# tum-vision/dvo_slam

Measured on NVIDIA H100. Metric: frame-pair alignments/sec @640x480x5-level, higher is better.
Workload: dtype f32

## Files before the change

### dvo_slam_b200/csrc/stages.cuh

```cuda
#pragma once
#include "common.cuh"
#include "f32x2.cuh"

namespace dvo_b200 {

constexpr unsigned kFullMask = 0xffffffffu;
constexpr int kConsumerWarps = kTileH;
constexpr int kCtaThreads = (kConsumerWarps + 1) * 32;
#ifndef DVO_WIN_COLS
#define DVO_WIN_COLS 152
#endif
#ifndef DVO_WIN_ROWS
#define DVO_WIN_ROWS 24
#endif
#ifndef DVO_STAGES
#define DVO_STAGES 2
#endif
constexpr int kWinCols = DVO_WIN_COLS;
constexpr int kWinRows = DVO_WIN_ROWS;
constexpr int kStages = DVO_STAGES;

__device__ __forceinline__ unsigned smem_u32(const void* p) { return (unsigned)__cvta_generic_to_shared(p); }
__device__ __forceinline__ void mbar_init(unsigned long long* bar, unsigned count) {
  asm volatile("mbarrier.init.shared::cta.b64 [%0], %1;" ::"r"(smem_u32(bar)), "r"(count) : "memory");
}
__device__ __forceinline__ void mbar_fence_init() { asm volatile("fence.mbarrier_init.release.cluster;" ::: "memory"); }
__device__ __forceinline__ void mbar_arrive(unsigned long long* bar) {
  asm volatile("{\n\t.reg .b64 st;\n\tmbarrier.arrive.release.cta.shared::cta.b64 st, [%0];\n\t}" ::"r"(smem_u32(bar)) : "memory");
}
__device__ __forceinline__ void mbar_arrive_expect_tx(unsigned long long* bar, unsigned bytes) {
  asm volatile("{\n\t.reg .b64 st;\n\tmbarrier.arrive.expect_tx.release.cta.shared::cta.b64 st, [%0], %1;\n\t}" ::"r"(smem_u32(bar)),
               "r"(bytes)
               : "memory");
}
#ifndef DVO_TRYWAIT_HINT_NS
#define DVO_TRYWAIT_HINT_NS 0
#endif
__device__ __forceinline__ bool mbar_try_wait(unsigned long long* bar, unsigned parity) {
  unsigned ok;
#if DVO_TRYWAIT_HINT_NS > 0
  asm volatile(
      "{\n\t.reg .pred p;\n\tmbarrier.try_wait.parity.acquire.cta.shared::cta.b64 p, [%1], %2, %3;\n\tselp.u32 %0, 1, 0, p;\n\t}"
      : "=r"(ok)
      : "r"(smem_u32(bar)), "r"(parity), "r"((unsigned)DVO_TRYWAIT_HINT_NS)
      : "memory");
#else
  asm volatile(
      "{\n\t.reg .pred p;\n\tmbarrier.try_wait.parity.acquire.cta.shared::cta.b64 p, [%1], %2;\n\tselp.u32 %0, 1, 0, p;\n\t}"
      : "=r"(ok)
      : "r"(smem_u32(bar)), "r"(parity)
      : "memory");
#endif
  return ok != 0;
}
__device__ __forceinline__ void mbar_wait(unsigned long long* bar, unsigned parity, int* error_flag) {
  unsigned spins = 0;
  while (!mbar_try_wait(bar, parity)) {
    if (((++spins) & 0xfffu) == 0u) {
      if (*reinterpret_cast<volatile int*>(error_flag)) break;
      if (spins > (1u << 24)) { atomicExch(error_flag, 2); break; }
    }
  }
}
__device__ __forceinline__ bool mbar_try_wait_s(unsigned bar, unsigned parity) {
  unsigned ok;
#if DVO_TRYWAIT_HINT_NS > 0
  asm volatile(
      "{\n\t.reg .pred p;\n\tmbarrier.try_wait.parity.acquire.cta.shared::cta.b64 p, [%1], %2, %3;\n\tselp.u32 %0, 1, 0, p;\n\t}"
      : "=r"(ok)
      : "r"(bar), "r"(parity), "r"((unsigned)DVO_TRYWAIT_HINT_NS)
      : "memory");
#else
  asm volatile(
      "{\n\t.reg .pred p;\n\tmbarrier.try_wait.parity.acquire.cta.shared::cta.b64 p, [%1], %2;\n\tselp.u32 %0, 1, 0, p;\n\t}"
      : "=r"(ok)
      : "r"(bar), "r"(parity)
      : "memory");
#endif
  return ok != 0;
}
__device__ __forceinline__ void mbar_wait_s(unsigned bar, unsigned parity, int* error_flag) {
  unsigned spins = 0;
  while (!mbar_try_wait_s(bar, parity)) {
    if (((++spins) & 0xfffu) == 0u) {
      if (*reinterpret_cast<volatile int*>(error_flag)) break;
      if (spins > (1u << 24)) { atomicExch(error_flag, 2); break; }
    }
  }
}
__device__ __forceinline__ void mbar_arrive_s(unsigned bar) {
  asm volatile("{\n\t.reg .b64 st;\n\tmbarrier.arrive.release.cta.shared::cta.b64 st, [%0];\n\t}" ::"r"(bar) : "memory");
}
__device__ __forceinline__ int4 lds_i4(unsigned addr) {
  int4 v;
  asm volatile("ld.shared.v4.b32 {%0, %1, %2, %3}, [%4];" : "=r"(v.x), "=r"(v.y), "=r"(v.z), "=r"(v.w) : "r"(addr));
  return v;
// ... 21 lines not shown
  asm volatile("ld.shared.v2.f32 {%0, %1}, [%2];" : "=f"(v.x), "=f"(v.y) : "r"(addr));
  return v;
}

__device__ __forceinline__ unsigned pin(unsigned v) { asm volatile("" : "+r"(v)); return v; }
__device__ __forceinline__ int pin(int v) { asm volatile("" : "+r"(v)); return v; }
__device__ __forceinline__ float pin(float v) { asm volatile("" : "+f"(v)); return v; }
template <typename T>
__device__ __forceinline__ const T* pin(const T* p) { asm volatile("" : "+l"(p)); return p; }

struct __align__(16) TileDesc {
  int skip;
  int origin;
  int ulo, ucount;
  int vlo, vcount;
  int exact;
  int pad_;
};
struct __align__(128) StageBuf {
  float2 ref0[kTileH][kTileW];
  float tx[kTileW];
  float2 ref1[kTileH][kTileW];
  float2 win[kWinRows][kWinCols];
};
static_assert(offsetof(StageBuf, tx) == kRecTx * sizeof(float2) && offsetof(StageBuf, ref1) == kRecP1 * sizeof(float2) &&
              offsetof(StageBuf, win) == kRecF2 * sizeof(float2), "StageBuf must mirror the reference tile record");
struct TilePipe {
  StageBuf buf[kStages];
  unsigned long long full[kStages], empty[kStages];
  TileDesc desc[kStages];
};
static_assert(sizeof(TileDesc) == 32 && offsetof(TilePipe, desc) % 16 == 0, "TileDesc is read as two 16-byte words");

#ifdef DVO_PIPE_TIMING
struct PipeTiming {
  unsigned long long wait_full_a = 0, wait_full_b = 0, wait_empty = 0, produce = 0, rounds_a = 0, rounds_b = 0;
  unsigned long long tiles = 0, tiles_inexact = 0, tiles_skipped = 0, slow_rounds = 0, rounds = 0;
  bool on = false;
};
#define DVO_CLOCK(tm) ((tm).on ? clock64() : 0)
#define DVO_ADD(tm, field, v) do { if ((tm).on) (tm).field += (v); } while (0)
#else
struct PipeTiming {};
#define DVO_CLOCK(tm) 0ll
#define DVO_ADD(tm, field, v) do { } while (0)
#endif

struct LevelGeom {
  int w, h, n, pitch;
  int nbands, nstrips;
  int strip0, strip_step, nmine;
};

struct StageConsts {
  f2 k0, k1, k2, k3;
  float k8, k9, k10, k11;
  f2 Pa, Pb;
  f2 cgh, cg, fxyh;
  float c_i, ubx, uby;
  int first_iteration;
};

__device__ __forceinline__ void load_stage_consts(const PairState& st, const PairLevel& pl, int w, int h, bool weights_from_prev,
                                                  StageConsts& c) {
  float kt[12], P[4];
#pragma unroll
  for (int i = 0; i < 12; ++i) kt[i] = __ldcg(&st.kt[i]);
#pragma unroll
  for (int i = 0; i < 4; ++i) P[i] = weights_from_prev ? __ldcg(&st.precision_prev[i]) : __ldcg(&st.precision[i]);
  c.k0 = pk(kt[0], kt[4]); c.k1 = pk(kt[1], kt[5]); c.k2 = pk(kt[2], kt[6]); c.k3 = pk(kt[3], kt[7]);
  c.k8 = kt[8]; c.k9 = kt[9]; c.k10 = kt[10]; c.k11 = kt[11];
  c.Pa = pk(P[0], P[1]); c.Pb = pk(P[2], P[3]);
  const float cgx = __fdiv_rn(__fmul_rn(0.5f, pl.cfx), 255.0f), cgy = __fdiv_rn(__fmul_rn(0.5f, pl.cfy), 255.0f);
  c.cg = pk(cgx, cgy);
  c.cgh = pk(0.5f * cgx, 0.5f * cgy);
  c.fxyh = pk(0.5f * pl.cfx, 0.5f * pl.cfy);
  c.c_i = 1.0f / 255.0f;
  c.ubx = pin((float)(w - 2)); c.uby = pin((float)(h - 2));
  c.first_iteration = __ldcg(&st.iteration) == 0;
}

template <bool kStageB>
__device__ __noinline__ void produce_tiles(TilePipe& tp, const PairLevel& pl, const LevelGeom& g, const StageConsts& c, unsigned tbase,
                                           int ntiles, int* error_flag, PipeTiming& tm) {
  const int lane = threadIdx.x & 31, sub = lane >> 3;
  const float2* cur = kStageB ? pl.c3 : pl.c0;
  int s_issue = g.strip0, b_issue = 0;
  for (int i0 = 0; i0 < ntiles; i0 += 4) {
    const long long tp0 = DVO_CLOCK(tm);
    unsigned wordA, wordD;
    {
      const int ii = min(i0 + sub, ntiles - 1);
      const int sd = ii / g.nbands;
      const int s = g.strip0 + sd * g.strip_step, b = ii - sd * g.nbands;
      const int y0 = s * kTileH, rows = min(kTileH, g.h - y0);
      const int x0 = b * kTileW, bw = min(kTileW, g.w - x0);
      const float2 zr = __ldg(pl.rrange + (size_t)s * g.nbands + b);
      const float txc = __ldg(pl.rtmpl + ((lane & 1) ? x0 + bw - 1 : x0));
      const float tyc = __ldg(pl.rtmpl + g.w + ((lane & 2) ? y0 + rows - 1 : y0));
      const bool has_depth = zr.x <= zr.y;
      const float z = (lane & 4) ? zr.y : zr.x;
      const float px = txc * z, py = tyc * z;
      const f2 XY = fma2(c.k0, bc(px), fma2(c.k1, bc(py), fma2(c.k2, bc(z), c.k3)));
      const float Zt = fmaf(c.k8, px, fmaf(c.k9, py, fmaf(c.k10, z, c.k11)));
      const float iz = 1.0f / Zt;
      float umin = lo(XY) * iz, vmin = hi(XY) * iz, umax = umin, vmax = vmin;
      const bool front_lane = Zt > 1e-6f && umin == umin && vmin == vmin;
#pragma unroll
      for (int off = 1; off < 8; off <<= 1) {
        umin = fminf(umin, __shfl_xor_sync(kFullMask, umin, off)); umax = fmaxf(umax, __shfl_xor_sync(kFullMask, umax, off));
        vmin = fminf(vmin, __shfl_xor_sync(kFullMask, vmin, off)); vmax = fmaxf(vmax, __shfl_xor_sync(kFullMask, vmax, off));
      }
      const bool front = ((__ballot_sync(kFullMask, front_lane) >> (sub * 8)) & 0xffu) == 0xffu;
      umin = fmaxf(umin, -8.f); vmin = fmaxf(vmin, -8.f); umax = fminf(umax, (float)g.w + 8.f); vmax = fminf(vmax, (float)g.h + 8.f);
      int skip = 0, exact = 0, ncols = 0, nrows = 0, bx0 = 0, row_lo = 0;
      if (!has_depth) {
        skip = 1;
      } else if (!front) {
      } else if (umax < -1.f || vmax < -1.f || umin > (float)g.w || vmin > (float)g.h) {
        skip = 1;
      } else {
        const int col_lo = max((int)floorf(umin) - 2, 0), col_hi = min((int)floorf(umax) + 3, g.w - 1);
        row_lo = max((int)floorf(vmin) - 2, -1);
        const int row_hi = min((int)floorf(vmax) + 3, g.h);
        bx0 = col_lo & ~1;
        ncols = (col_hi + 2 - bx0) & ~1;
        bool whole = true;
        if (ncols > kWinCols) { bx0 += ((ncols - kWinCols) / 2) & ~1; ncols = kWinCols; whole = false; }
        nrows = row_hi - row_lo + 1;
        if (nrows > kWinRows) { row_lo += (nrows - kWinRows) / 2; nrows = kWinRows; whole = false; }
        if (ncols < 4 || nrows < 4) { ncols = 0; nrows = 0; bx0 = 0; row_lo = 0; }
        else exact = whole ? 1 : 0;
      }
      wordA = (unsigned)skip | ((unsigned)exact << 1) | ((unsigned)ncols << 2) | ((unsigned)nrows << 10);
      wordD = (unsigned)bx0 | ((unsigned)(row_lo + 1) << 16);
    }
    DVO_ADD(tm, produce, DVO_CLOCK(tm) - tp0);
    const int kmax = min(4, ntiles - i0);
    for (int k = 0; k < kmax; ++k) {
      const unsigned t = tbase + (unsigned)(i0 + k);
      const int bufi = t % kStages;
      StageBuf& sb = tp.buf[bufi];
      const unsigned wa = __shfl_sync(kFullMask, wordA, k * 8), wd = __shfl_sync(kFullMask, wordD, k * 8);
      const int s = s_issue, b = b_issue;
      if (++b_issue == g.nbands) { b_issue = 0; s_issue += g.strip_step; }
      const int skip = (int)(wa & 1u), ncols = (int)((wa >> 2) & 0xffu), nrows = (int)(wa >> 10);
      const int win_bx0 = (int)(wd & 0xffffu), win_row_lo = (int)(wd >> 16) - 1;
      TileDesc d;
      d.skip = skip; d.exact = (int)((wa >> 1) & 1u); d.pad_ = 0;
      d.origin = 0; d.ulo = 0; d.ucount = 0; d.vlo = 0; d.vcount = 0;
      if (ncols) {
        d.origin = (win_row_lo * kWinCols + win_bx0) * 8;
        d.ulo = win_bx0 == 0 ? 0 : win_bx0 + 1;
        const int uhi = (win_bx0 + ncols - 1 >= g.w - 1) ? g.w - 2 : win_bx0 + ncols - 3;
        d.ucount = max(uhi - d.ulo + 1, 0);
        d.vlo = win_row_lo + 1;
        d.vcount = max(nrows - 3, 0);
      }
      const unsigned win_row_bytes = (unsigned)ncols * 8u;
      const unsigned rec_bytes = (unsigned)(kStageB ? kRecF2 : kRecP1) * 8u;
      const unsigned total = skip ? 0u : rec_bytes + (unsigned)nrows * win_row_bytes;
      const long long tp1 = DVO_CLOCK(tm);
      mbar_wait(&tp.empty[bufi], ((t / kStages) & 1u) ^ 1u, error_flag);
      DVO_ADD(tm, wait_empty, DVO_CLOCK(tm) - tp1);
      DVO_ADD(tm, tiles, 1); DVO_ADD(tm, tiles_inexact, (!d.skip && !d.exact) ? 1 : 0); DVO_ADD(tm, tiles_skipped, d.skip ? 1 : 0);
      if (lane == 0) {
        tp.desc[bufi] = d;
        if (total) mbar_arrive_expect_tx(&tp.full[bufi], total);
        else mbar_arrive(&tp.full[bufi]);
      }
      __syncwarp();
      if (!skip) {
        if (lane < nrows) {
          const int yy = min(max(win_row_lo + lane, 0), g.h - 1);
          bulk_g2s(&sb.win[lane][0], cur + (size_t)yy * g.pitch + win_bx0, win_row_bytes, &tp.full[bufi]);
        }
        if (lane == 31) bulk_g2s(&sb.ref0[0][0], pl.r0 + (size_t)(s * g.nbands + b) * kRecF2, rec_bytes, &tp.full[bufi]);
      }
    }
  }
}

struct PixelProjection {
  f2 f, gq;
  float Zt;
  int u0, v0;
  bool inb;
};

__device__ __forceinline__ PixelProjection project_pixel(float tx, float ty, float z, const StageConsts& c) {
  PixelProjection p;
  const f2 pxy = mul2(pk(tx, ty), bc(z));
  const float px = lo(pxy), py = hi(pxy);
  const f2 XY = fma2(c.k0, bc(px), fma2(c.k1, bc(py), fma2(c.k2, bc(z), c.k3)));
  p.Zt = __fmaf_rn(c.k8, px, __fmaf_rn(c.k9, py, __fmaf_rn(c.k10, z, c.k11)));
  f2 uv = mul2(XY, bc(rcp_rn(p.Zt)));
  const float u = lo(uv), v = hi(uv);
  p.inb = u >= 0.f && u <= c.ubx && v >= 0.f && v <= c.uby;
  uv = p.inb ? uv : bc(0.f);
  const f2 t = add2_rz(uv, bc(8388608.0f));
  p.f = sub2(uv, sub2(t, bc(8388608.0f)));
  p.gq = sub2(bc(1.0f), p.f);
  p.u0 = __float_as_int(lo(t)) - 0x4b000000;
  p.v0 = __float_as_int(hi(t)) - 0x4b000000;
  return p;
}

#define DVO_BLEND2(fu, fv, gu, gv, c00, c10, c01, c11) \
  fma2(bc(fv), fma2(bc(fu), c11, mul2(bc(gu), c01)), mul2(bc(gv), fma2(bc(fu), c10, mul2(bc(gu), c00))))

__device__ __forceinline__ f2 ld_f2(const float2* p) { const float2 v = *p; return pk(v.x, v.y); }

struct WinView {
  bool exact;
  unsigned base;
  unsigned safe;
  const float2* plane;
  int ulo, ucount, vlo, vcount;
  int w, h, pitch;
};
constexpr int kWinRowBytes = kWinCols * 8;

struct Taps4 { f2 c00, c10, c01, c11; };
struct Taps12 { f2 c00, c10, c01, c11, l0, l1, r0, r1, t0, t1, b0, b1; };

__device__ __forceinline__ void gather_taps4(const WinView& wv, int u0, int v0, bool inb, bool hit, Taps4& t) {
  const bool miss = inb && !hit;
  const unsigned sa = (inb && hit) ? wv.base + (unsigned)(v0 * kWinCols + u0) * 8u : wv.safe;
  const float2* p = miss ? wv.plane + (size_t)v0 * wv.pitch + u0 : reinterpret_cast<const float2*>(__cvta_shared_to_generic(sa));
  const int rp = miss ? wv.pitch : kWinCols;
  t.c00 = ld_f2(p); t.c10 = ld_f2(p + 1); t.c01 = ld_f2(p + rp); t.c11 = ld_f2(p + rp + 1);
}
__device__ __forceinline__ void gather_taps12(const WinView& wv, int u0, int v0, bool inb, bool hit, Taps12& t) {
  const bool miss = inb && !hit;
  const unsigned sa = (inb && hit) ? wv.base + (unsigned)(v0 * kWinCols + u0) * 8u : wv.safe;
  const float2* p = miss ? wv.plane + (size_t)v0 * wv.pitch + u0 : reinterpret_cast<const float2*>(__cvta_shared_to_generic(sa));
  const int rp = miss ? wv.pitch : kWinCols;
  const int up = (miss && v0 == 0) ? 0 : -rp;
  const int dn = (miss && v0 + 2 > wv.h - 1) ? rp : 2 * rp;
  const int dl = u0 > 0 ? 1 : 0, dr = u0 + 2 <= wv.w - 1 ? 2 : 1;
  t.c00 = ld_f2(p); t.c10 = ld_f2(p + 1); t.c01 = ld_f2(p + rp); t.c11 = ld_f2(p + rp + 1);
  t.t0 = ld_f2(p + up); t.t1 = ld_f2(p + up + 1); t.b0 = ld_f2(p + dn); t.b1 = ld_f2(p + dn + 1);
  t.l0 = ld_f2(p - dl); t.l1 = ld_f2(p + rp - dl); t.r0 = ld_f2(p + dr); t.r1 = ld_f2(p + rp + dr);
}

__device__ __forceinline__ float depth_sigma(float z) {
  const float s = __fsub_rn(z, 0.4f);
  return __fmaf_rn(__fmul_rn(0.0019f, s), s, 0.0012f);
}

template <bool kExact>
__device__ __forceinline__ bool residual_pixel(const PixelProjection& p, const WinView& wv, float Ir, float z, const StageConsts& c,
                                               float& ei, float& ez) {
  bool hit = true, any_miss = false;
  if (!kExact && !wv.exact) {
    hit = (unsigned)(p.u0 - wv.ulo) < (unsigned)wv.ucount && (unsigned)(p.v0 - wv.vlo) < (unsigned)wv.vcount;
    any_miss = __any_sync(kFullMask, p.inb && !hit);
  }
  f2 c00, c10, c01, c11;
  if (!any_miss) {
    const unsigned a = p.inb ? wv.base + (unsigned)(p.v0 * kWinCols + p.u0) * 8u : wv.safe;
    c00 = lds_f2<0>(a); c10 = lds_f2<8>(a); c01 = lds_f2<kWinRowBytes>(a); c11 = lds_f2<kWinRowBytes + 8>(a);
  } else {
    Taps4 t;
    gather_taps4(wv, p.u0, p.v0, p.inb, hit, t);
// ... 200 lines not shown
    const f2 ss = pk(s, __int_as_float(__float_as_int(s) ^ st.psign));
    st.acc0 = fma2(ss, bc(st.po0), st.acc0); st.acc1 = fma2(ss, bc(st.po1), st.acc1); st.acc2 = fma2(ss, bc(st.po2), st.acc2);
  }
  const float a0 = xi * xi, a1 = xi * xz, a2 = xz * xz;
  const float s = (v && next) ? w + wn : 0.f;
  const f2 ss = pk(s, __int_as_float(__float_as_int(s) ^ sg));
  st.acc0 = fma2(ss, bc(a0), st.acc0); st.acc1 = fma2(ss, bc(a1), st.acc1); st.acc2 = fma2(ss, bc(a2), st.acc2);
  st.pend = v && !next;
  st.pw = w; st.po0 = a0; st.po1 = a1; st.po2 = a2; st.psign = sg;
  st.cnt += __popc(m);
}

__device__ __forceinline__ void scale_state_export(ScaleState& st, int lane, float* seg_out) {
  float all0 = lo(st.acc0), alt0 = hi(st.acc0), all1 = lo(st.acc1), alt1 = hi(st.acc1), all2 = lo(st.acc2), alt2 = hi(st.acc2);
#pragma unroll
  for (int off = 16; off > 0; off >>= 1) {
    all0 += __shfl_xor_sync(kFullMask, all0, off); alt0 += __shfl_xor_sync(kFullMask, alt0, off);
    all1 += __shfl_xor_sync(kFullMask, all1, off); alt1 += __shfl_xor_sync(kFullMask, alt1, off);
    all2 += __shfl_xor_sync(kFullMask, all2, off); alt2 += __shfl_xor_sync(kFullMask, alt2, off);
  }
  if (lane == 0) {
    seg_out[0] = __int_as_float(st.cnt);
    seg_out[1] = (float)(0.5 * ((double)all0 + (double)alt0)); seg_out[2] = (float)(0.5 * ((double)all1 + (double)alt1));
    seg_out[3] = (float)(0.5 * ((double)all2 + (double)alt2));
    seg_out[4] = (float)(0.5 * ((double)all0 - (double)alt0)); seg_out[5] = (float)(0.5 * ((double)all1 - (double)alt1));
    seg_out[6] = (float)(0.5 * ((double)all2 - (double)alt2));
    seg_out[7] = st.wfirst;
    if (st.cnt == 0) { seg_out[8] = 0.f; seg_out[9] = 0.f; seg_out[10] = 0.f; seg_out[11] = 0.f; }
  }
  if (st.pend) {
    seg_out[8] = st.pw; seg_out[9] = st.po0; seg_out[10] = st.po1; seg_out[11] = st.po2;
  }
}

__device__ __forceinline__ WinView make_view(unsigned bufs, const int4& d0, const int4& d1, const float2* plane, int w, int h, int pitch) {
  WinView wv;
  const unsigned w0 = bufs + (unsigned)offsetof(StageBuf, win);
  wv.base = pin(w0 - (unsigned)d0.y);
  wv.safe = pin(w0 + (unsigned)((kWinCols + 1) * 8));
  wv.plane = plane;
  wv.exact = d1.z != 0;
  wv.ulo = d0.z; wv.ucount = d0.w; wv.vlo = d1.x; wv.vcount = d1.y;
  wv.w = w; wv.h = h; wv.pitch = pitch;
  return wv;
}


template <bool kExact, bool kFirst>
__device__ __forceinline__ void stage_a_rounds(const WinView& wv, int bw, unsigned refa, unsigned txa, float ty, const StageConsts& c,
                                               ScaleState& ss, int lane, unsigned lt_mask) {
  static_assert(kTileW % 64 == 0, "the exact loop takes whole pairs of rounds");
  const int nr = kExact ? kTileW / 32 : (bw + 31) >> 5;
  const int xlim = bw - lane;
  const bool first = kExact ? kFirst : c.first_iteration != 0;
#pragma unroll 1
  for (int r = 0; r < nr; r += 2, refa += 512, txa += 256) {
    const bool second = kExact || r + 1 < nr;
    const f2 rz0 = lds_f2_at(refa);
    const f2 rz1 = second ? lds_f2_at(refa + 256) : pk(0.f, __int_as_float(0x7fc00000));
    const float tx0 = lds_f32(txa), tx1 = second ? lds_f32(txa + 128) : 0.f;
    float z0 = hi(rz0), z1 = hi(rz1);
    if (!kExact && bw < kTileW) {
      z0 = (r * 32 < xlim) ? z0 : __int_as_float(0x7fc00000);
      z1 = (r * 32 + 32 < xlim) ? z1 : __int_as_float(0x7fc00000);
    }
    const PixelProjection p0 = project_pixel(tx0, ty, z0, c);
    const PixelProjection p1 = project_pixel(tx1, ty, z1, c);
    float ei0, ez0, ei1, ez1;
    const bool v0 = residual_pixel<kExact>(p0, wv, lo(rz0), z0, c, ei0, ez0);
    const bool v1 = residual_pixel<kExact>(p1, wv, lo(rz1), z1, c, ei1, ez1);
    const float w0 = student_weight(c, first, ei0, ez0), w1 = student_weight(c, first, ei1, ez1);
    scale_round32(ss, lane, lt_mask, v0, w0, ei0, ez0);
    scale_round32(ss, lane, lt_mask, v1, w1, ei1, ez1);
  }
}
__device__ __forceinline__ void stage_a_run(TilePipe& tp, const PairLevel& pl, const LevelGeom& g, const StageConsts& c,
                                            float* row_exports, unsigned& tile_count, int* error_flag, PipeTiming& tm) {
  const int lane = threadIdx.x & 31, q = threadIdx.x >> 5;
  const unsigned lt_mask = (1u << lane) - 1u;
  const int ntiles = g.nmine * g.nbands;
  const unsigned tbase = tile_count;
  tile_count += ntiles;
  if (q == kConsumerWarps) {
    produce_tiles<false>(tp, pl, g, c, tbase, ntiles, error_flag, tm);
    return;
  }
  int i = 0;
  const unsigned tp_s = pin(smem_u32(&tp));
  const unsigned my_ref = pin((unsigned)(offsetof(StageBuf, ref0) + (q * kTileW + lane) * 8));
  const unsigned my_tx = pin((unsigned)(offsetof(StageBuf, tx) + lane * 4));
  const int gw = pin(g.w), gh = pin(g.h), gnb = pin(g.nbands), gpitch = g.pitch;
  for (int sk = 0, s = g.strip0; sk < g.nmine; ++sk, s += g.strip_step) {
    const int y = s * kTileH + q;
    const bool row_ok = y < gh;
    const float ty = __ldg(pl.rtmpl + gw + min(y, gh - 1));
    ScaleState ss;
    scale_state_init(ss);
    for (int b = 0; b < gnb; ++b, ++i) {
      const unsigned t = tbase + i;
      const unsigned bufi = t % kStages;
      const int x0 = b * kTileW, bw = min(kTileW, gw - x0);
      const long long tw0 = DVO_CLOCK(tm);
      mbar_wait_s(tp_s + (unsigned)offsetof(TilePipe, full) + bufi * 8u, (t / kStages) & 1u, error_flag);
      DVO_ADD(tm, wait_full_a, DVO_CLOCK(tm) - tw0);
      const unsigned bufs = tp_s + bufi * (unsigned)sizeof(StageBuf);
      const int4 d0 = lds_i4(tp_s + (unsigned)offsetof(TilePipe, desc) + bufi * 32u);
      if (row_ok && !d0.x) {
        const int4 d1 = lds_i4(tp_s + (unsigned)offsetof(TilePipe, desc) + bufi * 32u + 16u);
        const WinView wv = make_view(bufs, d0, d1, pl.c0, gw, gh, gpitch);
        const unsigned refa = bufs + my_ref, txa = bufs + my_tx;
        if (wv.exact && bw == kTileW) {
          if (c.first_iteration) stage_a_rounds<true, true>(wv, bw, refa, txa, ty, c, ss, lane, lt_mask);
          else stage_a_rounds<true, false>(wv, bw, refa, txa, ty, c, ss, lane, lt_mask);
        } else {
          stage_a_rounds<false, false>(wv, bw, refa, txa, ty, c, ss, lane, lt_mask);
        }
      }
      __syncwarp();
      if (lane == 0) mbar_arrive_s(tp_s + (unsigned)offsetof(TilePipe, empty) + bufi * 8u);
    }
    if (row_ok) scale_state_export(ss, lane, row_exports + (size_t)y * kSegExportFloats);
  }
}

struct StageBConsts {
  float P00, P01, P10, P11;
  float l, wd0, wd1;
};

constexpr int kNormalValues = 28;

constexpr int kTriValues = 21;
__host__ __device__ constexpr int tri(int r, int c) { return r * 6 - r * (r - 1) / 2 + (c - r); }
struct StageBAcc {
  float A[kTriValues];
  float b[6];
  float llsum;
};

__device__ __forceinline__ void stage_b_init(StageBAcc& a) {
#pragma unroll
  for (int i = 0; i < kTriValues; ++i) a.A[i] = 0.f;
#pragma unroll
  for (int i = 0; i < 6; ++i) a.b[i] = 0.f;
  a.llsum = 0.f;
}

__device__ __forceinline__ void stage_b_rank1(StageBAcc& acc, const f2 V[3], float wd, float s) {
  const float v[6] = {lo(V[0]), hi(V[0]), lo(V[1]), hi(V[1]), lo(V[2]), hi(V[2])};
  float u[6];
#pragma unroll
  for (int r = 0; r < 6; ++r) u[r] = __fmul_rn(v[r], wd);
#pragma unroll
  for (int r = 0; r < 6; ++r) {
#pragma unroll
    for (int c = r; c < 6; ++c) acc.A[tri(r, c)] = __fmaf_rn(u[r], v[c], acc.A[tri(r, c)]);
  }
#pragma unroll
  for (int r = 0; r < 6; ++r) acc.b[r] = __fmaf_rn(u[r], s, acc.b[r]);
}

__device__ __forceinline__ void stage_b_pixel(StageBAcc& acc, const StageBConsts& c, float wgt, bool keep, float ei, float ez, f2 G,
                                              f2 H, float z, float tx, float ty) {
  const float d = (ei * c.P00 + ez * c.P10) * ei + (ei * c.P01 + ez * c.P11) * ez;
  acc.llsum += __log2f(keep ? fmaf(0.2f, d, 1.0f) : 1.0f);
  const float px = tx * z, py = ty * z;
  const float zi = rcp_fast(z), zs = zi * zi;
// ... 23 lines not shown
__device__ __forceinline__ void halving_step(float (&a)[16], int lane) {
  const bool up = (lane & kHalf) != 0;
#pragma unroll
  for (int j = 0; j < kHalf; ++j) {
    const float mine = up ? a[kHalf + j] : a[j];
    const float send = up ? a[j] : a[kHalf + j];
    a[j] = mine + __shfl_xor_sync(kFullMask, send, kHalf);
  }
}

__device__ __forceinline__ void flush_row_partial(const StageBAcc& acc, int lane, float* row_out) {
  float a[16];
  const bool up = (lane & 16) != 0;
#pragma unroll
  for (int j = 0; j < 16; ++j) {
    const float mine = up ? stage_b_value(acc, 16 + j) : stage_b_value(acc, j);
    const float send = up ? stage_b_value(acc, j) : stage_b_value(acc, 16 + j);
    a[j] = mine + __shfl_xor_sync(kFullMask, send, 16);
  }
  halving_step<8>(a, lane);
  halving_step<4>(a, lane);
  halving_step<2>(a, lane);
  halving_step<1>(a, lane);
  if (lane < kNormalValues) row_out[lane] = a[0];
}

struct RecordDump {
  float* planes;
  int n;
};
__device__ __noinline__ void dump_record(const RecordDump& dump, size_t i, bool valid, f2 E, f2 G, f2 H, float z) {
  const float nanv = __int_as_float(0x7fc00000);
  float* p = dump.planes + i;
  const size_t n = (size_t)dump.n;
  p[0] = valid ? lo(E) : nanv; p[n] = valid ? hi(E) : nanv;
  p[2 * n] = valid ? lo(G) : nanv; p[3 * n] = valid ? hi(G) : nanv;
  p[4 * n] = valid ? lo(H) : nanv; p[5 * n] = valid ? hi(H) : nanv;
  p[6 * n] = valid ? z : nanv;
}

template <bool kExact, bool kFirst, bool kDump>
__device__ __forceinline__ void stage_b_rounds(const WinView& wv, int bw, unsigned refa, unsigned txa, float ty, const StageConsts& c,
                                               const StageBConsts& cb, StageBAcc& acc, bool cta_has_tail, int& rank, int keep_rank,
                                               const RecordDump& dump, size_t pix, int lane, unsigned lt_mask, PipeTiming& tm) {
  const int nr = kExact ? kTileW / 32 : (bw + 31) >> 5;
  const int xlim = bw - lane;
  const bool first = kExact ? kFirst : c.first_iteration != 0;
#pragma unroll 1
  for (int r = 0; r < nr; ++r, refa += 256, txa += 128) {
    const f2 rz = lds_f2_at(refa);
    const f2 gr = lds_f2<sizeof(float2) * kRecP1>(refa);
    const float tx = lds_f32(txa);
    float z = hi(rz);
    if (!kExact && bw < kTileW) z = (r * 32 < xlim) ? z : __int_as_float(0x7fc00000);
    const PixelProjection p = project_pixel(tx, ty, z, c);
    f2 E, G, H;
    const bool valid = record_pixel<kExact>(p, wv, lo(rz), z, gr, c, E, G, H);
    DVO_ADD(tm, rounds, 1); DVO_ADD(tm, slow_rounds, kExact ? 0 : 1);
    bool keep = valid;
    if (!kExact && cta_has_tail) {
      const unsigned m = __ballot_sync(kFullMask, valid);
      keep = valid && (rank + __popc(m & lt_mask)) < keep_rank;
      rank += __popc(m);
    }
    if (kDump && r * 32 < xlim) dump_record(dump, pix + r * 32, valid, E, G, H, z);
    const float ei = valid ? lo(E) : 0.f, ez = valid ? hi(E) : 0.f;
    const float wall = student_weight(c, first, ei, ez);
    const float wgt = valid ? wall : 0.f;
    stage_b_pixel(acc, cb, wgt, keep, ei, ez, valid ? G : bc(0.f), valid ? H : bc(0.f), valid ? z : 1.0f, valid ? tx : 0.f, ty);
  }
}

template <bool kDump>
__device__ __forceinline__ void stage_b_run(TilePipe& tp, const PairLevel& pl, const LevelGeom& g, const StageConsts& c,
                                            const StageBConsts& cb, const int* row_base, const int* strip_base, long long n_keep,
                                            const RecordDump& dump, float* row_partial, unsigned& tile_count, int* error_flag,
                                            PipeTiming& tm) {
  const int lane = threadIdx.x & 31, q = threadIdx.x >> 5;
  const unsigned lt_mask = (1u << lane) - 1u;
  const int ntiles = g.nmine * g.nbands;
  const unsigned tbase = tile_count;
  tile_count += ntiles;
  if (q == kConsumerWarps) {
    produce_tiles<true>(tp, pl, g, c, tbase, ntiles, error_flag, tm);
    return;
  }
  int i = 0;
  const unsigned tp_s = pin(smem_u32(&tp));
  const unsigned my_ref = (unsigned)(offsetof(StageBuf, ref0) + (q * kTileW + lane) * 8);
  const unsigned my_tx = (unsigned)(offsetof(StageBuf, tx) + lane * 4);
  const int gw = g.w, gh = g.h, gnb = g.nbands, gpitch = g.pitch;
  for (int sk = 0, s = g.strip0; sk < g.nmine; ++sk, s += g.strip_step) {
    const int y = s * kTileH + q;
    const bool row_ok = y < gh;
    const float ty = __ldg(pl.rtmpl + gw + min(y, gh - 1));
    const long long sbase = __ldcg(strip_base + s);
    const bool cta_has_tail = (long long)__ldcg(strip_base + s + 1) > n_keep;
    const int keep_rank = (int)max(min(n_keep - sbase, (long long)0x7fffffff), (long long)-1);
    int rank = 0;
    if (cta_has_tail && row_ok) rank = __ldcg(row_base + y);
    StageBAcc acc;
    stage_b_init(acc);
    for (int b = 0; b < gnb; ++b, ++i) {
      const unsigned t = tbase + i;
      const unsigned bufi = t % kStages;
      const int x0 = b * kTileW, bw = min(kTileW, gw - x0);
      const long long tw0 = DVO_CLOCK(tm);
      mbar_wait_s(tp_s + (unsigned)offsetof(TilePipe, full) + bufi * 8u, (t / kStages) & 1u, error_flag);
      DVO_ADD(tm, wait_full_b, DVO_CLOCK(tm) - tw0);
      const unsigned bufs = tp_s + bufi * (unsigned)sizeof(StageBuf);
      const int4 d0 = lds_i4(tp_s + (unsigned)offsetof(TilePipe, desc) + bufi * 32u);
      if (row_ok && !d0.x) {
        const int4 d1 = lds_i4(tp_s + (unsigned)offsetof(TilePipe, desc) + bufi * 32u + 16u);
        const WinView wv = make_view(bufs, d0, d1, pl.c3, gw, gh, gpitch);
        const unsigned refa = bufs + my_ref, txa = bufs + my_tx;
        const size_t pix = (size_t)y * gw + x0 + lane;
        if (wv.exact && bw == kTileW && !cta_has_tail) {
          if (c.first_iteration)
            stage_b_rounds<true, true, kDump>(wv, bw, refa, txa, ty, c, cb, acc, cta_has_tail, rank, keep_rank, dump, pix, lane, lt_mask, tm);
          else
            stage_b_rounds<true, false, kDump>(wv, bw, refa, txa, ty, c, cb, acc, cta_has_tail, rank, keep_rank, dump, pix, lane, lt_mask, tm);
        } else {
          stage_b_rounds<false, false, kDump>(wv, bw, refa, txa, ty, c, cb, acc, cta_has_tail, rank, keep_rank, dump, pix, lane, lt_mask, tm);
        }
      } else if (kDump && row_ok) {
        for (int xl = lane; xl < bw; xl += 32) dump_record(dump, (size_t)y * gw + x0 + xl, false, bc(0.f), bc(0.f), bc(0.f), 0.f);
      }
      __syncwarp();
      if (lane == 0) mbar_arrive_s(tp_s + (unsigned)offsetof(TilePipe, empty) + bufi * 8u);
    }
    if (row_ok) flush_row_partial(acc, lane, row_partial + (size_t)y * kNormalValues);
  }
}

__device__ __forceinline__ void load_stage_b_consts(const PairState& st, StageBConsts& c) {
  c.P00 = __ldcg(&st.precision[0]); c.P01 = __ldcg(&st.precision[1]); c.P10 = __ldcg(&st.precision[2]); c.P11 = __ldcg(&st.precision[3]);
  c.l = c.P01 / c.P00;
  c.wd0 = c.P00;
  c.wd1 = c.P11 - c.P01 * c.l;
}

}
```

### dvo_slam_b200/csrc/tracker.cu

```cuda
#include "common.cuh"
#include "stages.cuh"

#include <cstdio>
#include <cstring>
#include <limits>
#include <cmath>
#include <cstdlib>
#include <algorithm>

namespace dvo_b200 {

namespace {

constexpr unsigned kFull = 0xffffffffu;
constexpr int kEndWarps = 4;

struct LevelLaunch {
  int w, h, n, pitch;
  int nbands, nstrips;
  int level_index;
  int level_id;
  int max_iterations;
  int first_level;
  int use_initial_estimate;
// ... 183 lines not shown
    iteration += 1;
  } else {
    for (int i = 0; i < 6; ++i) x[i] = st.x[i];
  }
  phase(2);
  double m = 0; bool nanx = false;
  for (int i = 0; i < 6; ++i) { m = fmax(m, fabs(x[i])); nanx |= x[i] != x[i]; }
  const bool big = !nanx && m > lp.precision;
  const bool exceeded = iteration >= lp.max_iterations;
  const bool level_done = !(accept && big && !exceeded);
  SE3d inc, estimate_new;
  if (!level_done) {
    inc = se3_exp(x);
    estimate_new = se3_mul(inc, st.estimate);
    double T[16];
    se3_matrix(estimate_new, T);
    for (int j = 0; j < 4; ++j) {
      const float t0 = (float)T[j], t1 = (float)T[4 + j], t2 = (float)T[8 + j];
      st.kt[j] = __fadd_rn(__fmul_rn(pl.cfx, t0), __fmul_rn(pl.cox, t2));
      st.kt[4 + j] = __fadd_rn(__fmul_rn(pl.cfy, t1), __fmul_rn(pl.coy, t2));
      st.kt[8 + j] = t2;
    }
    st.iteration = iteration;
  } else {
    st.level_active = 0;
  }
  phase(3);
  if (tcrit) { unsigned long long tc1; asm volatile("mov.u64 %0, %globaltimer;" : "=l"(tc1)); atomicAdd(tcrit + 7, tc1 - tc0); }
  release();
  phase(4);

  LevelSummary& ls = st.levels[lp.level_index];
  st.ll = ll;
  st.nll_cur = -(double)ll;
  st.prior_cur = lp.mu * sq;
  st.last_error = last_error;
  st.error = error;
  for (int i = 0; i < 36; ++i) st.A[i] = A[i];
  for (int i = 0; i < 6; ++i) st.b[i] = bvec[i];
  if (!accept) {
    st.initial = st.initial_old; st.estimate = st.estimate_old;
    st.termination = DVO_B200_TERM_LOG_LIKELIHOOD_DECREASED;
    log_iteration(ilog, max_log, pair, st, it_id, lp.level_id, false);
  } else {
    for (int i = 0; i < 6; ++i) st.x[i] = x[i];
    for (int i = 0; i < 36; ++i) st.A_done[i] = A[i];
    for (int i = 0; i < 6; ++i) st.A_done[i * 6 + i] += lp.mu;
    st.nll_done = st.nll_cur; st.prior_done = st.prior_cur; st.have_done = 1;
    ls.last_inc_n = st.n; ls.last_inc_nll = st.nll_cur;
    log_iteration(ilog, max_log, pair, st, it_id, lp.level_id, true);
    st.iteration = iteration;
  }
  if (level_done) {
    if (!nanx && m <= lp.precision) st.termination = DVO_B200_TERM_INCREMENT_TOO_SMALL;
    if (exceeded) st.termination = DVO_B200_TERM_ITERATIONS_EXCEEDED;
    ls.termination = st.termination;
    int need = (st.termination == DVO_B200_TERM_LOG_LIKELIHOOD_DECREASED ||
                st.termination == DVO_B200_TERM_TOO_FEW_CONSTRAINTS) ? 2 : 1;
    ls.has_inc = ls.num_iterations >= need;
    if (active) atomicSub(active, 1);
  } else {
    st.inc = inc;
    st.initial_old = st.initial;
    st.initial = se3_mul(se3_inverse(inc), st.initial);
    st.estimate_old = st.estimate;
    st.estimate = estimate_new;
  }
  phase(5);
}

struct SquadState {
  int pair;
  unsigned arrive;
  unsigned phase;
  int pad_[29];
};

struct LevelTail {
  SegCombineSmem comb;
  PairEndSmem end;
  int s_flag[2];
};
constexpr size_t kLevelSmemBytes = sizeof(TilePipe) + sizeof(LevelTail);

constexpr int kMaxSeg = 4;
struct Segment {
  const PairLevel* pls;
  float* row_exports;
  int* row_base;
  double* strip_exports;
  int* strip_base;
  float* row_partial;
  double* strip_partial;
  SquadState* squads;
  int* queue;
  int* ready;
  int* ready_tail;
  int* arrivals;
  int cyclic;
  int pair_begin;
  int npairs_seg;
  unsigned long long* dbg2;
  unsigned long long* dbg;
  int nlev;
  int g, nsquads;
  int strips_per_cta[kMaxLevels];
  LevelLaunch lp[kMaxLevels];
};

struct PersistentArgs {
  PairState* states;
  int* error_flag;
  dvo_b200_iteration_stats* ilog;
  int max_log;
  const double* T_init;
  int skip_begin;
  float* dump;
  int npairs;
  int nseg;
  Segment seg[kMaxSeg];
};

__device__ __forceinline__ unsigned long long global_ns() {
  unsigned long long t;
  asm volatile("mov.u64 %0, %globaltimer;" : "=l"(t));
  return t;
}

__device__ __forceinline__ unsigned ld_acquire_u32(const unsigned* p) {
  unsigned v;
  asm volatile("ld.acquire.gpu.global.u32 %0, [%1];" : "=r"(v) : "l"(p) : "memory");
  return v;
}

__device__ __forceinline__ bool squad_arrive(SquadState* sq, unsigned episode, int g, int* s_flag) {
  __syncthreads();
  if (threadIdx.x == 0) {
    __threadfence();
    unsigned old = atomicAdd(&sq->arrive, 1u);
    int last = old == (episode + 1u) * (unsigned)g - 1u;
    if (last) __threadfence();
    s_flag[0] = last;
  }
  __syncthreads();
  return s_flag[0] != 0;
}
__device__ __forceinline__ void squad_release(SquadState* sq, unsigned episode) {
  __threadfence();
  atomicExch(&sq->phase, episode + 1u);
}
__device__ __forceinline__ void squad_wait(SquadState* sq, unsigned episode, int* error_flag) {
  if (threadIdx.x == 0) {
    unsigned spins = 0;
    while (ld_acquire_u32(&sq->phase) < episode + 1u) {
      __nanosleep(100);
      if (((++spins) & 4095u) == 0u) {
        if (*reinterpret_cast<volatile int*>(error_flag)) break;
        if (spins > (1u << 25)) { atomicExch(error_flag, 1); break; }
      }
    }
  }
  __syncthreads();
}

__global__ void __launch_bounds__(kCtaThreads, 2)
k_level_persistent(const __grid_constant__ PersistentArgs a) {
// ... 50 lines not shown
      if (threadIdx.x == 0) {
        int p = atomicAdd(S.queue, 1);
        if (p >= S.npairs_seg) p = -1;
        else if (fused && si >= 1) {
          unsigned spins = 0;
          int v;
          while ((v = (int)ld_acquire_u32(reinterpret_cast<const unsigned*>(S.ready + p))) == 0) {
            __nanosleep(200);
            if (((++spins) & 4095u) == 0u) {
              if (*reinterpret_cast<volatile int*>(a.error_flag)) break;
              if (spins > (1u << 24)) { atomicExch(a.error_flag, 1); break; }
            }
          }
          p = v - 1;
        }
        sq->pair = p;
        squad_release(sq, episode);
      }
    } else {
      squad_wait(sq, episode, a.error_flag);
    }
    __syncthreads();
    ++episode;
    DVO_TOCK(6);
    const int pair = __ldcg(&sq->pair);
    if (pair < 0 || *reinterpret_cast<volatile int*>(a.error_flag)) break;
    PairState& st = a.states[pair];

    for (int li = 0; li < S.nlev; ++li) {
    const LevelLaunch& lp = S.lp[li];
    const PairLevel pl = S.pls[(size_t)li * a.npairs + pair];
    LevelGeom geo;
    geo.w = lp.w; geo.h = lp.h; geo.n = lp.n; geo.pitch = lp.pitch; geo.nbands = lp.nbands; geo.nstrips = lp.nstrips;
    if (S.cyclic) {
      const int g_eff = min(S.g, lp.nstrips);
      geo.strip0 = min(rank, lp.nstrips); geo.strip_step = g_eff;
      geo.nmine = rank < g_eff ? (lp.nstrips - rank + g_eff - 1) / g_eff : 0;
    } else {
      geo.strip0 = min(rank * S.strips_per_cta[li], lp.nstrips); geo.strip_step = 1;
      geo.nmine = min(geo.strip0 + S.strips_per_cta[li], lp.nstrips) - geo.strip0;
    }
    if (!a.skip_begin) {
      if (squad_arrive(sq, episode, S.g, lt.s_flag)) {
        if (threadIdx.x == 0) {
          level_begin(st, pl, a.T_init, pair, lp);
          squad_release(sq, episode);
        }
      } else {
        squad_wait(sq, episode, a.error_flag);
      }
      __syncthreads();
      ++episode;
      DVO_TOCK(6);
    }

    for (;;) {
      {
        StageConsts c;
        load_stage_consts(st, pl, lp.w, lp.h, false, c);
        const long long ts0 = DVO_CLOCK(tm);
        stage_a_run(tp, pl, geo, c, row_exports, tile_count, a.error_flag, tm);
        DVO_ADD(tm, rounds_a, DVO_CLOCK(tm) - ts0);
      }
      __syncthreads();
      for (int j = threadIdx.x; j < geo.nmine; j += kCtaThreads) {
        const int sj = geo.strip0 + j * geo.strip_step;
        combine_strip_rows(row_exports, sj * kTileH, min(sj * kTileH + kTileH, lp.h), row_base, strip_exports + (size_t)sj * kStripExportDoubles);
      }
      DVO_TOCK(0);
      if (squad_arrive(sq, episode, S.g, lt.s_flag)) {
        DVO_TOCK(2);
        if (warp == 0) {
          pair_mid_warp(st, pair, strip_exports, strip_base, lp.nstrips, nullptr, lp, a.ilog, a.max_log, lt.comb);
          if (lane == 0) squad_release(sq, episode);
        }
        __syncthreads();
        DVO_TOCK(4);
      } else {
        squad_wait(sq, episode, a.error_flag);
        DVO_TOCK(2);
      }
      __syncthreads();
      ++episode;
      if (!__ldcg(&st.level_active) || *reinterpret_cast<volatile int*>(a.error_flag)) break;

      {
        StageConsts c;
        load_stage_consts(st, pl, lp.w, lp.h, true, c);
        StageBConsts cb;
        load_stage_b_consts(st, cb);
        const long long n_keep = __ldcg(&st.n_keep);
        RecordDump dump;
        dump.planes = a.dump; dump.n = lp.n;
        const long long ts0 = DVO_CLOCK(tm);
        if (a.dump) stage_b_run<true>(tp, pl, geo, c, cb, row_base, strip_base, n_keep, dump, row_partial, tile_count, a.error_flag, tm);
        else stage_b_run<false>(tp, pl, geo, c, cb, row_base, strip_base, n_keep, dump, row_partial, tile_count, a.error_flag, tm);
        DVO_ADD(tm, rounds_b, DVO_CLOCK(tm) - ts0);
      }
      __syncthreads();
      for (int it = threadIdx.x; it < geo.nmine * kNormalValues; it += kCtaThreads) {
        const int j = it / kNormalValues, i = it - j * kNormalValues;
        const int sj = geo.strip0 + j * geo.strip_step;
        const int nrow = min(kTileH, lp.h - sj * kTileH);
        const float* rp = row_partial + (size_t)sj * kTileH * kNormalValues + i;
        float r[kTileH];
#pragma unroll
        for (int k = 0; k < kTileH; ++k) r[k] = k < nrow ? __ldcg(rp + (size_t)k * kNormalValues) : 0.f;
        double v = 0.0;
#pragma unroll
        for (int k = 0; k < kTileH; ++k) v += (double)r[k];
        strip_partial[(size_t)sj * kNormalValues + i] = v;
      }
      DVO_TOCK(1);
      if (squad_arrive(sq, episode, S.g, lt.s_flag)) {
        DVO_TOCK(3);
        pair_end_cta(st, pl, pair, strip_partial, lp.nstrips, nullptr, lp, a.ilog, a.max_log, lt.end, [&] { squad_release(sq, episode); }, S.dbg2 ? S.dbg2 + 64 : nullptr);
        __syncthreads();
        DVO_TOCK(5);
      } else {
        squad_wait(sq, episode, a.error_flag);
        DVO_TOCK(3);
      }
      __syncthreads();
      ++episode;
      if (!__ldcg(&st.level_active) || *reinterpret_cast<volatile int*>(a.error_flag)) break;
    }
    if (*reinterpret_cast<volatile int*>(a.error_flag)) break;
    }
    if (fused && si == 0 && threadIdx.x == 0) {
      int k = 1;
      while (k + 1 < a.nseg && pair >= a.seg[k + 1].pair_begin) ++k;
      __threadfence();
      const int slot = atomicAdd(a.seg[k].ready_tail, 1);
      asm volatile("st.release.gpu.global.u32 [%0], %1;" :: "l"(a.seg[k].ready + slot), "r"(pair + 1) : "memory");
    }
  }
  if (timing) {
    t_acc[7] = global_ns() - t_start;
    for (int i = 0; i < 8; ++i) atomicAdd(S.dbg + i, t_acc[i]);
  }
#ifdef DVO_PIPE_TIMING
  if (tm.on) {
    if (warp == 0) { atomicAdd(S.dbg + 8, tm.rounds_a); atomicAdd(S.dbg + 9, tm.wait_full_a); atomicAdd(S.dbg + 10, tm.rounds_b); atomicAdd(S.dbg + 11, tm.wait_full_b); }
    else { atomicAdd(S.dbg + 12, tm.produce); atomicAdd(S.dbg + 13, tm.wait_empty); atomicAdd(S.dbg + 14, tm.rounds_a); atomicAdd(S.dbg + 15, tm.rounds_b); }
    if (warp == 0) { atomicAdd(S.dbg2 + 3, tm.rounds); atomicAdd(S.dbg2 + 4, tm.slow_rounds); }
    else { atomicAdd(S.dbg2 + 0, tm.tiles); atomicAdd(S.dbg2 + 1, tm.tiles_inexact); atomicAdd(S.dbg2 + 2, tm.tiles_skipped); }
  }
  if (timing) { atomicMax(S.dbg2 + 5, t_acc[7]); atomicMin(S.dbg2 + 6, t_acc[7]); }
#endif
  }
#undef DVO_TICK
#undef DVO_TOCK
}

__global__ void k_finalize(PairState* states, dvo_b200_result* results, int npairs) {
  int p = blockIdx.x * blockDim.x + threadIdx.x;
  if (p >= npairs) return;
  PairState& st = states[p];
  dvo_b200_result& r = results[p];
  const double nan = __longlong_as_double(0x7ff8000000000000LL);
  se3_matrix(se3_inverse(st.estimate), r.transformation);
  bool ok = st.have_done == 1 && st.termination != DVO_B200_TERM_TOO_FEW_CONSTRAINTS;
  for (int i = 0; i < 36; ++i) r.information[i] = ok ? st.A_done[i] * 0.008 * 0.008 : nan;
  r.log_likelihood = ok ? st.nll_done + st.prior_done : nan;
  r.num_levels = st.num_levels;
  r.num_iterations_total = st.num_iterations_total;
  for (int l = 0; l < kMaxLevels; ++l) {
// ... 548 lines not shown
```

Before: 18320.

## Prefetch first stage-B tiles during stage A and shrink window to fit two CTAs

After issuing all stage-A tiles, the producer warp now also issues the first kStages stage-B tile loads, so these bulk copies overlap the mid-pair reduction and barrier instead of starting only after it. When the level terminates, consumers drain and release the prefetched buffers so the pipeline parity stays consistent. The shared-memory window is reduced from 152x24 to 144x21, with a static_assert that two CTAs fit per SM, presumably to raise occupancy. Risks include the stage-B tiles being fetched with pre-update constants, wasted bandwidth on terminating iterations, and a smaller window producing more inexact tiles.

Measured after the change: 18700 (median of 6 runs). 2.1% higher.

```diff
diff --git a/dvo_slam_b200/csrc/stages.cuh b/dvo_slam_b200/csrc/stages.cuh
--- a/dvo_slam_b200/csrc/stages.cuh
+++ b/dvo_slam_b200/csrc/stages.cuh
@@ -8,10 +8,10 @@
 constexpr int kConsumerWarps = kTileH;
 constexpr int kCtaThreads = (kConsumerWarps + 1) * 32;
 #ifndef DVO_WIN_COLS
-#define DVO_WIN_COLS 152
+#define DVO_WIN_COLS 144
 #endif
 #ifndef DVO_WIN_ROWS
-#define DVO_WIN_ROWS 24
+#define DVO_WIN_ROWS 21
 #endif
 #ifndef DVO_STAGES
 #define DVO_STAGES 2
@@ -199,15 +199,16 @@
 
 template <bool kStageB>
 __device__ __noinline__ void produce_tiles(TilePipe& tp, const PairLevel& pl, const LevelGeom& g, const StageConsts& c, unsigned tbase,
-                                           int ntiles, int* error_flag, PipeTiming& tm) {
+                                           int ibegin, int iend, int* error_flag, PipeTiming& tm) {
   const int lane = threadIdx.x & 31, sub = lane >> 3;
   const float2* cur = kStageB ? pl.c3 : pl.c0;
-  int s_issue = g.strip0, b_issue = 0;
-  for (int i0 = 0; i0 < ntiles; i0 += 4) {
+  const int sd0 = ibegin / g.nbands;
+  int s_issue = g.strip0 + sd0 * g.strip_step, b_issue = ibegin - sd0 * g.nbands;
+  for (int i0 = ibegin; i0 < iend; i0 += 4) {
     const long long tp0 = DVO_CLOCK(tm);
     unsigned wordA, wordD;
     {
-      const int ii = min(i0 + sub, ntiles - 1);
+      const int ii = min(i0 + sub, iend - 1);
       const int sd = ii / g.nbands;
       const int s = g.strip0 + sd * g.strip_step, b = ii - sd * g.nbands;
       const int y0 = s * kTileH, rows = min(kTileH, g.h - y0);
@@ -253,7 +254,7 @@
       wordD = (unsigned)bx0 | ((unsigned)(row_lo + 1) << 16);
     }
     DVO_ADD(tm, produce, DVO_CLOCK(tm) - tp0);
-    const int kmax = min(4, ntiles - i0);
+    const int kmax = min(4, iend - i0);
     for (int k = 0; k < kmax; ++k) {
       const unsigned t = tbase + (unsigned)(i0 + k);
       const int bufi = t % kStages;
@@ -298,6 +299,25 @@
   }
 }
 
+__device__ __forceinline__ int stage_b_prefetch_tiles(const LevelGeom& g) { return min(kStages, g.nmine * g.nbands); }
+
+__device__ __noinline__ void produce_stage_a(TilePipe& tp, const PairLevel& pl, const LevelGeom& g, const StageConsts& c, unsigned tbase,
+                                             int* error_flag, PipeTiming& tm) {
+  const int ntiles = g.nmine * g.nbands;
+  produce_tiles<false>(tp, pl, g, c, tbase, 0, ntiles, error_flag, tm);
+  produce_tiles<true>(tp, pl, g, c, tbase + ntiles, 0, stage_b_prefetch_tiles(g), error_flag, tm);
+}
+
+__device__ __noinline__ void drop_stage_b_prefetch(TilePipe& tp, unsigned tbase, int npre, int* error_flag) {
+  if ((threadIdx.x >> 5) == kConsumerWarps) return;
+  for (int i = 0; i < npre; ++i) {
+    const unsigned t = tbase + (unsigned)i;
+    mbar_wait(&tp.full[t % kStages], (t / kStages) & 1u, error_flag);
+    __syncwarp();
+    if ((threadIdx.x & 31) == 0) mbar_arrive(&tp.empty[t % kStages]);
+  }
+}
+
 struct PixelProjection {
   f2 f, gq;
   float Zt;
@@ -664,7 +684,7 @@
   const unsigned tbase = tile_count;
   tile_count += ntiles;
   if (q == kConsumerWarps) {
-    produce_tiles<false>(tp, pl, g, c, tbase, ntiles, error_flag, tm);
+    produce_stage_a(tp, pl, g, c, tbase, error_flag, tm);
     return;
   }
   int i = 0;
@@ -854,7 +874,7 @@
   const unsigned tbase = tile_count;
   tile_count += ntiles;
   if (q == kConsumerWarps) {
-    produce_tiles<true>(tp, pl, g, c, tbase, ntiles, error_flag, tm);
+    produce_tiles<true>(tp, pl, g, c, tbase, stage_b_prefetch_tiles(g), ntiles, error_flag, tm);
     return;
   }
   int i = 0;
diff --git a/dvo_slam_b200/csrc/tracker.cu b/dvo_slam_b200/csrc/tracker.cu
--- a/dvo_slam_b200/csrc/tracker.cu
+++ b/dvo_slam_b200/csrc/tracker.cu
@@ -289,6 +289,7 @@
   int s_flag[2];
 };
 constexpr size_t kLevelSmemBytes = sizeof(TilePipe) + sizeof(LevelTail);
+static_assert(2 * (kLevelSmemBytes + 1024) <= 164 * 1024, "two level-kernel CTAs must fit in the 164 KB shared-memory configuration");
 
 constexpr int kMaxSeg = 4;
 struct Segment {
@@ -505,7 +506,12 @@
       }
       __syncthreads();
       ++episode;
-      if (!__ldcg(&st.level_active) || *reinterpret_cast<volatile int*>(a.error_flag)) break;
+      if (!__ldcg(&st.level_active) || *reinterpret_cast<volatile int*>(a.error_flag)) {
+        const int npre = stage_b_prefetch_tiles(geo);
+        drop_stage_b_prefetch(tp, tile_count, npre, a.error_flag);
+        tile_count += npre;
+        break;
+      }
 
       {
         StageConsts c;
```
